# KRLabsOrg/verbatim-rag

Measured on AMD Instinct MI355X. Metric: query x chunk span-extractions/sec @512tok (ModernBERT-base extractor, chunks/s), higher is better.
Workload: dtype bf16

## Files before the change

### verbatim-rag_amd/csrc/qkv_attn.hip

```cpp
#include "qkv_attn.h"

#include <cstdlib>
#include <type_traits>

#ifdef VRAG_DEBUG_API
#define VRAG_DBG(bit) ((p.debug_flags & (bit)) != 0)
#else
#define VRAG_DBG(bit) false
#endif

namespace vrag {

constexpr int QA_WB = 192 * 128;
constexpr int QA_XOFF = 2 * QA_WB;
constexpr int QA_TAB = 131072;
constexpr int QA_MU = QA_TAB, QA_RS = QA_TAB + 2048, QA_LS = QA_TAB + 4096;
constexpr int QA_CA = QA_TAB + 5120, QA_SA = QA_CA + 4096, QA_CB = QA_SA + 4096, QA_SB = QA_CB + 2048;
constexpr int QA_SMEM = QA_SB + 2048;
constexpr int QA_V_OFF = 65536;

constexpr float QA_LAZY = 8.0f;
__device__ __forceinline__ float max3f(float a, float b, float c) { return __builtin_fmaxf(__builtin_fmaxf(a, b), c); }

template <int N>
__device__ __forceinline__ void wait_vm() {
  asm volatile("s_waitcnt vmcnt(%0)" ::"n"(N) : "memory");
}

template <bool LOCAL, bool FOLD, typename T>
__global__ __launch_bounds__(512, 2) void qkv_attn_kernel(const QkvAttnParams p) {
  typedef typename Op<T>::v4 V4;
  typedef typename Op<T>::v8 V8;
  extern __shared__ __attribute__((aligned(16))) char smem[];
  const int tid = threadIdx.x;
  const int lane = tid & 63;
  const int wave = uniform(tid >> 6);
  const int g = lane >> 4, l15 = lane & 15;
  const int H = p.H, Tp = p.Tp, nh = p.nh;
  const int xcd = blockIdx.x & 7, slot = blockIdx.x >> 3;
  const int grp = (slot / nh) * 8 + xcd, head = slot % nh;
  if (grp >= p.n_groups) return;
  const int4 wd = p.groups[grp * 8 + wave];
  const int wrow0 = uniform(wd.x), S = uniform(wd.y), kbase = uniform(wd.z);
  const int srow0 = wave * 64;
  const int qrow0 = (wave - kbase) * 64;
  const bool active = qrow0 < S;
  const T* X = reinterpret_cast<const T*>(p.x);
  const T* Wh = reinterpret_cast<const T*>(p.w) + (size_t)head * 192 * H;

  unsigned voffX[2], voffW[3];
#pragma unroll
  for (int par = 0; par < 2; ++par) {
    const int r = par * 8 + (lane >> 3);
    voffX[par] = (unsigned)(r * H + (((lane & 7) ^ ((r >> 1) & 7)) << 3)) * 2u;
  }
#pragma unroll
  for (int i = 0; i < 3; ++i) {
    const int row = wave * 24 + i * 8 + (lane >> 3);
    voffW[i] = (unsigned)(row * H + (((lane & 7) ^ ((row >> 1) & 7)) << 3)) * 2u;
  }
  const char* const Xw = reinterpret_cast<const char*>(X + (size_t)wrow0 * H);
  const char* const Wb = reinterpret_cast<const char*>(Wh);
  char* const xbuf = smem + QA_XOFF + wave * 8192;
  auto dma_w = [&](int kt, int buf, int i) {
    if (VRAG_DBG(4)) return;
    unsigned vo = voffW[i];
    asm volatile("" : "+v"(vo));
    glds16(Wb + kt * 128 + vo, smem + buf * QA_WB + (wave * 24 + i * 8) * 128);
  };
  auto dma_x = [&](int kt, int i) {
    if (!active || VRAG_DBG(4)) return;
    unsigned vo = voffX[i & 1];
    asm volatile("" : "+v"(vo));
    glds16(Xw + ((size_t)(i >> 1) * 16 * H + kt * 64) * 2 + vo, xbuf + i * 1024);
  };

  if (!VRAG_DBG(4)) {
    if (FOLD && lane < 16) {
      glds16(p.ln_mu + min(wrow0 + lane * 4, Tp - 4), smem + QA_MU + srow0 * 4);
      glds16(p.ln_rstd + min(wrow0 + lane * 4, Tp - 4), smem + QA_RS + srow0 * 4);
    }
    if (FOLD && wave == 2) glds16(p.ln_s + head * 192 + lane * 4, smem + QA_LS);
    if (wave == 2 || wave == 3) {
      const float* tab = wave == 2 ? p.rope_cos : p.rope_sin;
#pragma unroll
      for (int i = 0; i < 2; ++i) {
        const int r = i * 8 + (lane >> 3);
        glds16(tab + min(r, p.rope_rows - 1) * 32 + (((lane & 7) ^ ((r >> 1) & 7)) << 2), smem + (wave == 2 ? QA_CB : QA_SB) + i * 1024);
      }
    }
    if (wave == 4 || wave == 5) {
      const float* tab = wave == 4 ? p.rope_cos : p.rope_sin;
#pragma unroll
      for (int i = 0; i < 4; ++i)
        glds16(tab + (size_t)min(16 * (i * 8 + (lane >> 3)), p.rope_rows - 1) * 32 + (lane & 7) * 4, smem + (wave == 4 ? QA_CA : QA_SA) + i * 1024);
    }
  }

  f32x4 acc[12][4];
#pragma unroll
  for (int a = 0; a < 12; ++a)
#pragma unroll
    for (int c = 0; c < 4; ++c) acc[a][c] = f32x4{0.f, 0.f, 0.f, 0.f};

  const int KT = H >> 6;
  int fo[2];
#pragma unroll
  for (int s2 = 0; s2 < 2; ++s2) fo[s2] = l15 * 128 + ((((4 * s2 + g) ^ ((l15 >> 1) & 7))) << 4);
#ifdef VRAG_DEBUG_API
  const int probe = p.debug_flags;
#else
  int probe = 0;
  asm volatile("" : "+s"(probe));
#endif
  const bool mm = active && !(probe & 2);
#pragma unroll
  for (int i = 0; i < 3; ++i) dma_w(0, 0, i);
#pragma unroll
  for (int i = 0; i < 8; ++i) dma_x(0, i);
  for (int kt = 0; kt < KT; ++kt) {
    wait_vm<0>();
    __builtin_amdgcn_s_barrier();
    asm volatile("" ::: "memory");
    const char* sW = smem + (kt & 1) * QA_WB;
    const bool more = kt + 1 < KT;
    V8 xf[2][4], wa;
    if (mm) {
#pragma unroll
      for (int s2 = 0; s2 < 2; ++s2)
#pragma unroll
        for (int rt = 0; rt < 4; ++rt) xf[s2][rt] = *reinterpret_cast<const V8*>(xbuf + rt * 16 * 128 + fo[s2]);
      wa = *reinterpret_cast<const V8*>(sW + fo[0]);
    }
    asm volatile("s_waitcnt lgkmcnt(0)" ::: "memory");
    __builtin_amdgcn_sched_barrier(0);
    if (mm) {
#pragma unroll
      for (int it = 0; it < 24; ++it) {
        const int s2 = it / 12, nj = it % 12;
        V8 na = wa;
        if (it < 23) na = *reinterpret_cast<const V8*>(sW + ((it + 1) % 12) * 16 * 128 + fo[(it + 1) / 12]);
        __builtin_amdgcn_sched_barrier(0);
#pragma unroll
        for (int rt = 0; rt < 4; ++rt) {
          if (nj < 8) acc[nj][rt] = Op<T>::mfma16(wa, xf[s2][rt], acc[nj][rt]);
          else acc[nj][rt] = Op<T>::mfma16(xf[s2][rt], wa, acc[nj][rt]);
        }
        __builtin_amdgcn_sched_barrier(0);
        if (more && it < 11) {
          if (it < 3) dma_w(kt + 1, (kt + 1) & 1, it);
          else dma_x(kt + 1, it - 3);
        }
        __builtin_amdgcn_sched_barrier(0);
        wa = na;
      }
    } else if (more) {
#pragma unroll
      for (int i = 0; i < 3; ++i) dma_w(kt + 1, (kt + 1) & 1, i);
#pragma unroll
      for (int i = 0; i < 8; ++i) dma_x(kt + 1, i);
    }
  }
  __syncthreads();
  if (VRAG_DBG(16)) return;

  const float* l_mu = reinterpret_cast<const float*>(smem + QA_MU) + srow0;
  const float* l_rs = reinterpret_cast<const float*>(smem + QA_RS) + srow0;
  const float* l_ls = reinterpret_cast<const float*>(smem + QA_LS);
#pragma unroll
  for (int db = 0; db < 4; ++db) {
    const int d = db * 16 + l15;
    const float lsv = FOLD ? l_ls[128 + d] : 0.f;
#pragma unroll
    for (int tp = 0; tp < 2; ++tp) {
      V8 vv;
#pragma unroll
      for (int a = 0; a < 2; ++a) {
        const int rt = 2 * tp + a;
        f32x4 m4 = {0.f, 0.f, 0.f, 0.f}, r4 = {1.f, 1.f, 1.f, 1.f};
        if constexpr (FOLD) {
          m4 = *reinterpret_cast<const f32x4*>(l_mu + rt * 16 + 4 * g);
          r4 = *reinterpret_cast<const f32x4*>(l_rs + rt * 16 + 4 * g);
        }
#pragma unroll
        for (int h = 0; h < 2; ++h) {
          const int r0 = 2 * h;
          const f32x2 v = pk_fma(f32x2{-m4[r0], -m4[r0 + 1]}, splat2(lsv), f32x2{acc[8 + db][rt][r0], acc[8 + db][rt][r0 + 1]}) * f32x2{r4[r0], r4[r0 + 1]};
#pragma unroll
          for (int e = 0; e < 2; ++e)
            vv[a * 4 + r0 + e] = qrow0 + rt * 16 + 4 * g + r0 + e < S ? Op<T>::to(v[e]) : (T)0.f;
        }
      }
      const int c = wave * 8 + tp * 4 + g;
      *reinterpret_cast<V8*>(smem + QA_V_OFF + d * 1024 + ((c ^ l15) << 4)) = vv;
    }
  }
  auto rope_rows = [&](int a0, int rt, int ls_off, float scale, V8 (&out)[2]) {
    const bool live = qrow0 + rt * 16 + l15 < S;
    const float mu = FOLD ? l_mu[rt * 16 + l15] : 0.f, rs = FOLD ? l_rs[rt * 16 + l15] : 1.f;
#pragma unroll
    for (int np = 0; np < 2; ++np) {
      const int dd = np * 16 + 4 * g;
      const f32x4 ca = *reinterpret_cast<const f32x4*>(smem + QA_CA + (((qrow0 >> 4) + rt) * 32 + dd) * 4);
      const f32x4 sa = *reinterpret_cast<const f32x4*>(smem + QA_SA + (((qrow0 >> 4) + rt) * 32 + dd) * 4);
      const int bsw = l15 * 128 + ((((dd >> 2) ^ ((l15 >> 1) & 7))) << 4);
      const f32x4 cb = *reinterpret_cast<const f32x4*>(smem + QA_CB + bsw);
      const f32x4 sb = *reinterpret_cast<const f32x4*>(smem + QA_SB + bsw);
      f32x4 l1 = {0.f, 0.f, 0.f, 0.f}, l2 = {0.f, 0.f, 0.f, 0.f};
      if constexpr (FOLD) {
        l1 = *reinterpret_cast<const f32x4*>(l_ls + ls_off + dd);
        l2 = *reinterpret_cast<const f32x4*>(l_ls + ls_off + 32 + dd);
      }
#pragma unroll
      for (int h = 0; h < 2; ++h) {
        const int j0 = 2 * h;
        f32x2 x1 = {acc[a0 + np][rt][j0], acc[a0 + np][rt][j0 + 1]}, x2 = {acc[a0 + 2 + np][rt][j0], acc[a0 + 2 + np][rt][j0 + 1]};
        if constexpr (FOLD) {
          x1 = pk_fma(splat2(-mu), f32x2{l1[j0], l1[j0 + 1]}, x1) * rs;
          x2 = pk_fma(splat2(-mu), f32x2{l2[j0], l2[j0 + 1]}, x2) * rs;
        }
        const f32x2 ca2 = {ca[j0], ca[j0 + 1]}, sa2 = {sa[j0], sa[j0 + 1]}, cb2 = {cb[j0], cb[j0 + 1]}, sb2 = {sb[j0], sb[j0 + 1]};
        const f32x2 c = pk_fma(-sa2, sb2, ca2 * cb2), sn = pk_fma(ca2, sb2, sa2 * cb2);
        const f32x2 o1 = pk_fma(-x2, sn, x1 * c) * scale, o2 = pk_fma(x1, sn, x2 * c) * scale;
#pragma unroll
        for (int e = 0; e < 2; ++e) {
          if constexpr (!std::is_same<T, bf16_t>::value) {
            out[0][np * 4 + j0 + e] = live ? Op<T>::to(o1[e]) : (T)0.f;
            out[1][np * 4 + j0 + e] = live ? Op<T>::to(o2[e]) : (T)0.f;
          } else {
            out[0][np * 4 + j0 + e] = Op<T>::to(o1[e]);
            out[1][np * 4 + j0 + e] = Op<T>::to(o2[e]);
          }
        }
      }
    }
  };
#pragma unroll
  for (int rt = 0; rt < 4; ++rt) {
    V8 kf[2];
    rope_rows(4, rt, 64, 1.0f, kf);
    const int row = srow0 + rt * 16 + l15;
#pragma unroll
    for (int s = 0; s < 2; ++s) *reinterpret_cast<V8*>(smem + row * 128 + (((4 * s + g) ^ ((row >> 1) & 7)) << 4)) = kf[s];
  }
  V8 qf[4][2];
#pragma unroll
  for (int rt = 0; rt < 4; ++rt) rope_rows(0, rt, 0, p.q_scale, qf[rt]);
  __syncthreads();

  f32x4 ot[4][4];
  f32x4 lo[4];
#pragma unroll
  for (int c = 0; c < 4; ++c) {
    lo[c] = f32x4{0.f, 0.f, 0.f, 0.f};
#pragma unroll
    for (int dt = 0; dt < 4; ++dt) ot[c][dt] = f32x4{0.f, 0.f, 0.f, 0.f};
  }
  float m_run[4] = {0.f, 0.f, 0.f, 0.f};
  bool seen[4] = {false, false, false, false};
  V8 ones;
#pragma unroll
  for (int j = 0; j < 8; ++j) ones[j] = (T)1.0f;
  const int W = p.window;
  int kt_lo = 0, kt_hi = (S - 1) >> 6;
  if constexpr (LOCAL) {
    kt_lo = max(0, qrow0 - W) >> 6;
    kt_hi = min(S - 1, qrow0 + 63 + W) >> 6;
  }
  const int ksw = (l15 >> 1) & 7;
  if (active && !VRAG_DBG(1)) {
    for (int kt = kt_lo; kt <= kt_hi; ++kt) {
      bool cut[2][2];
#pragma unroll
      for (int u = 0; u < 2; ++u) {
        const int q_lo = qrow0 + 32 * u;
#pragma unroll
        for (int t2 = 0; t2 < 2; ++t2) {
          const int kh = kt * 64 + t2 * 32;
          bool outside = kh >= S || q_lo >= S;
          cut[u][t2] = kh + 31 >= S;
          if constexpr (LOCAL) {
            outside = outside || (kh + 31 < q_lo - W) || (kh > q_lo + 31 + W);
            cut[u][t2] = cut[u][t2] || (kh < q_lo + 31 - W) || (kh + 31 > q_lo + W);
          }
          cut[u][t2] = cut[u][t2] || outside;
        }
      }
      V8 pf[4][2];
      {
        f32x4 st[4][4];
#pragma unroll
        for (int c = 0; c < 4; ++c) {
          const float seed = -m_run[c];
#pragma unroll
          for (int kb = 0; kb < 4; ++kb) st[c][kb] = f32x4{seed, seed, seed, seed};
        }
#pragma unroll
        for (int kb = 0; kb < 4; ++kb) {
          const char* krow = smem + ((kbase + kt) * 64 + kb * 16 + l15) * 128;
          const V8 k0 = *reinterpret_cast<const V8*>(krow + ((g ^ ksw) << 4));
          const V8 k1 = *reinterpret_cast<const V8*>(krow + (((4 + g) ^ ksw) << 4));
#pragma unroll
          for (int c = 0; c < 4; ++c) {
            st[c][kb] = Op<T>::mfma16(k0, qf[c][0], st[c][kb]);
            st[c][kb] = Op<T>::mfma16(k1, qf[c][1], st[c][kb]);
          }
        }
        float mx[4];
#pragma unroll
        for (int c = 0; c < 4; ++c) {
          const int u = c >> 1;
          mx[c] = -INFINITY;
#pragma unroll
          for (int t2 = 0; t2 < 2; ++t2) {
            if (cut[u][t2]) {
              const int qi = qrow0 + 16 * c + l15;
              int lo_k = 0, hi_k = S - 1;
              if constexpr (LOCAL) {
                lo_k = max(0, qi - W);
                hi_k = min(S - 1, qi + W);
              }
              const unsigned span = hi_k >= lo_k ? (unsigned)(hi_k - lo_k) : 0u;
              int d0 = hi_k >= lo_k ? kt * 64 + t2 * 32 + 4 * g - lo_k : -100000;
              asm volatile("" : "+v"(d0));
#pragma unroll
              for (int h2 = 0; h2 < 2; ++h2)
#pragma unroll
                for (int r = 0; r < 4; ++r) {
                  const bool ok = (unsigned)(d0 + 16 * h2 + r) <= span;
                  st[c][2 * t2 + h2][r] = ok ? st[c][2 * t2 + h2][r] : -INFINITY;
                }
            }
            const f32x4& a = st[c][2 * t2];
            const f32x4& b2 = st[c][2 * t2 + 1];
            mx[c] = max3f(mx[c], max3f(a[0], a[1], a[2]), max3f(a[3], b2[0], b2[1]));
            mx[c] = max3f(mx[c], b2[2], b2[3]);
          }
        }
        bool move = false;
#pragma unroll
        for (int c = 0; c < 4; ++c) move = move || mx[c] > QA_LAZY || (!seen[c] && mx[c] > -INFINITY);
        if (__any(move)) {
#pragma unroll
          for (int c = 0; c < 4; ++c) {
            float m_all = fmaxf(mx[c], __shfl_xor(mx[c], 16, 64));
            m_all = fmaxf(m_all, __shfl_xor(m_all, 32, 64));
            const bool has = m_all > -INFINITY;
            const float delta = seen[c] ? fmaxf(m_all, 0.f) : (has ? m_all : 0.f);
            const float alpha = seen[c] ? __builtin_amdgcn_exp2f(-delta) : 1.0f;
            seen[c] = seen[c] || has;
            m_run[c] += delta;
#pragma unroll
            for (int kb = 0; kb < 4; ++kb)
#pragma unroll
              for (int r = 0; r < 4; ++r) st[c][kb][r] -= delta;
#pragma unroll
            for (int dt = 0; dt < 4; ++dt)
#pragma unroll
              for (int r = 0; r < 4; ++r) ot[c][dt][r] *= alpha;
#pragma unroll
            for (int r = 0; r < 4; ++r) lo[c][r] *= alpha;
          }
        }
#pragma unroll
        for (int c = 0; c < 4; ++c)
#pragma unroll
          for (int t2 = 0; t2 < 2; ++t2)
#pragma unroll
            for (int j = 0; j < 8; ++j) pf[c][t2][j] = (T)__builtin_amdgcn_exp2f(st[c][2 * t2 + (j >> 2)][j & 3]);
      }
#pragma unroll
      for (int t2 = 0; t2 < 2; ++t2) {
#pragma unroll
        for (int c = 0; c < 4; ++c) lo[c] = Op<T>::mfma16(ones, pf[c][t2], lo[c]);
#pragma unroll
        for (int dt = 0; dt < 4; ++dt) {
          const V8 vf = *reinterpret_cast<const V8*>(smem + QA_V_OFF + (dt * 16 + l15) * 1024 + ((((kbase + kt) * 8 + t2 * 4 + g) ^ l15) << 4));
#pragma unroll
          for (int c = 0; c < 4; ++c) ot[c][dt] = Op<T>::mfma16(vf, pf[c][t2], ot[c][dt]);
        }
      }
    }
  }
  __syncthreads();

  if (active) {
    char* stg = smem + wave * 8192;
#pragma unroll
    for (int rt = 0; rt < 4; ++rt) {
      const int row = rt * 16 + l15;
      const bool live = qrow0 + row < S;
      const float inv = live ? 1.0f / lo[rt][0] : 0.f;
#pragma unroll
      for (int db = 0; db < 4; ++db) {
        V4 o;
#pragma unroll
        for (int j = 0; j < 4; ++j) o[j] = live ? Op<T>::to(ot[rt][db][j] * inv) : (T)0.f;
        const int c16 = db * 2 + (g >> 1);
        *reinterpret_cast<V4*>(stg + row * 128 + ((c16 ^ (row & 7)) << 4) + ((g & 1) << 3)) = o;
      }
    }
#pragma unroll
    for (int it = 0; it < 8; ++it) {
      const int row = it * 8 + (lane >> 3), c16 = lane & 7;
      const f32x4 v = *reinterpret_cast<const f32x4*>(stg + row * 128 + ((c16 ^ (row & 7)) << 4));
      if (qrow0 + row < S && !VRAG_DBG(8)) store16_nt(reinterpret_cast<T*>(p.o) + (size_t)(wrow0 + row) * H + head * 64 + c16 * 8, v);
    }
  }
}

template <bool LOCAL, bool FOLD, typename T>
static hipError_t launch_t(const QkvAttnParams& p, hipStream_t stream) {
  static bool attr = false;
  if (!attr) {
    hipError_t e = hipFuncSetAttribute(reinterpret_cast<const void*>(&qkv_attn_kernel<LOCAL, FOLD, T>),
                                       hipFuncAttributeMaxDynamicSharedMemorySize, QA_SMEM);
    if (e != hipSuccess) return e;
    attr = true;
  }
  const int grid = ((p.n_groups + 7) / 8) * 8 * p.nh;
  hipLaunchKernelGGL((qkv_attn_kernel<LOCAL, FOLD, T>), dim3(grid), dim3(512), QA_SMEM, stream, p);
  return hipGetLastError();
}

hipError_t launch_qkv_attention(const QkvAttnParams& p, bool local, hipStream_t stream) {
  if (p.n_groups <= 0) return hipSuccess;
  if (p.H % 64 != 0 || p.H != p.nh * 64 || (size_t)p.Tp * p.H >= (size_t)1 << 31) return hipErrorInvalidValue;
  const bool fold = p.ln_mu != nullptr;
  if (p.op_dtype == kOpF16) {
    if (fold) return local ? launch_t<true, true, f16_t>(p, stream) : launch_t<false, true, f16_t>(p, stream);
    return local ? launch_t<true, false, f16_t>(p, stream) : launch_t<false, false, f16_t>(p, stream);
  }
  if (fold) return local ? launch_t<true, true, bf16_t>(p, stream) : launch_t<false, true, bf16_t>(p, stream);
  return local ? launch_t<true, false, bf16_t>(p, stream) : launch_t<false, false, bf16_t>(p, stream);
}

__global__ void permute_qkv_heads_kernel(const bf16_t* __restrict__ w, const float* __restrict__ s, int H, int nh,
                                         bf16_t* __restrict__ w_out, float* __restrict__ s_out) {
  const int orow = blockIdx.x;
  const int head = orow / 192, part = (orow % 192) / 64, d = orow % 64;
  const int src = part * H + head * 64 + d;
  for (int i = threadIdx.x; i < H; i += blockDim.x) w_out[(size_t)orow * H + i] = w[(size_t)src * H + i];
  if (threadIdx.x == 0 && s && s_out) s_out[orow] = s[src];
}

hipError_t permute_qkv_heads(const bf16_t* w, const float* s, int H, int nh, bf16_t* w_out, float* s_out, hipStream_t stream) {
  hipLaunchKernelGGL(permute_qkv_heads_kernel, dim3(3 * H), dim3(256), 0, stream, w, s, H, nh, w_out, s_out);
  return hipGetLastError();
}

int fused_pack_groups(const int* seq_row, const int* seq_len, int seq0, int seq1, int4* out) {
  int n = 0, used = 8;
  for (int s = seq0; s < seq1; ++s) {
    const int need = (seq_len[s] + 63) / 64;
    if (used + need > 8) {
      for (int w = 0; w < 8; ++w) out[n * 8 + w] = int4{0, 0, 0, 0};
      ++n;
      used = 0;
    }
    for (int j = 0; j < need; ++j) out[(n - 1) * 8 + used + j] = int4{seq_row[s] + 64 * j, seq_len[s], used, 0};
    used += need;
  }
  return n;
}

unsigned qkv_attn_f16_saturated(bool reset) { return f16_sat_take(reset); }
unsigned* qkv_attn_f16_flag_address() { return f16_sat_flag_address(); }

}
```

Baseline: 7860.

## Skip dead 32x32 sub-tiles at local-window edges and merge Q/K RoPE passes

The key-tile loop becomes a templated tile lambda that takes a compile-time live mask. For local attention, the first and last key tiles are peeled off and run with masks that drop MFMA, softmax and PV work for 32x32 quadrants wholly outside the window. Separately, RoPE for K and Q now runs in one pass per row tile, sharing the cos/sin table loads. Risks include more code size and register pressure from the extra instantiations, and the asm barrier on qf may change scheduling.

```diff
diff --git a/verbatim-rag_amd/csrc/qkv_attn.hip b/verbatim-rag_amd/csrc/qkv_attn.hip
--- a/verbatim-rag_amd/csrc/qkv_attn.hip
+++ b/verbatim-rag_amd/csrc/qkv_attn.hip
@@ -195,7 +195,7 @@
       *reinterpret_cast<V8*>(smem + QA_V_OFF + d * 1024 + ((c ^ l15) << 4)) = vv;
     }
   }
-  auto rope_rows = [&](int a0, int rt, int ls_off, float scale, V8 (&out)[2]) {
+  auto rope_rows = [&](int rt, V8 (&kout)[2], V8 (&qout)[2]) {
     const bool live = qrow0 + rt * 16 + l15 < S;
     const float mu = FOLD ? l_mu[rt * 16 + l15] : 0.f, rs = FOLD ? l_rs[rt * 16 + l15] : 1.f;
 #pragma unroll
@@ -206,46 +206,49 @@
       const int bsw = l15 * 128 + ((((dd >> 2) ^ ((l15 >> 1) & 7))) << 4);
       const f32x4 cb = *reinterpret_cast<const f32x4*>(smem + QA_CB + bsw);
       const f32x4 sb = *reinterpret_cast<const f32x4*>(smem + QA_SB + bsw);
-      f32x4 l1 = {0.f, 0.f, 0.f, 0.f}, l2 = {0.f, 0.f, 0.f, 0.f};
-      if constexpr (FOLD) {
-        l1 = *reinterpret_cast<const f32x4*>(l_ls + ls_off + dd);
-        l2 = *reinterpret_cast<const f32x4*>(l_ls + ls_off + 32 + dd);
-      }
 #pragma unroll
       for (int h = 0; h < 2; ++h) {
         const int j0 = 2 * h;
-        f32x2 x1 = {acc[a0 + np][rt][j0], acc[a0 + np][rt][j0 + 1]}, x2 = {acc[a0 + 2 + np][rt][j0], acc[a0 + 2 + np][rt][j0 + 1]};
-        if constexpr (FOLD) {
-          x1 = pk_fma(splat2(-mu), f32x2{l1[j0], l1[j0 + 1]}, x1) * rs;
-          x2 = pk_fma(splat2(-mu), f32x2{l2[j0], l2[j0 + 1]}, x2) * rs;
-        }
         const f32x2 ca2 = {ca[j0], ca[j0 + 1]}, sa2 = {sa[j0], sa[j0 + 1]}, cb2 = {cb[j0], cb[j0 + 1]}, sb2 = {sb[j0], sb[j0 + 1]};
         const f32x2 c = pk_fma(-sa2, sb2, ca2 * cb2), sn = pk_fma(ca2, sb2, sa2 * cb2);
-        const f32x2 o1 = pk_fma(-x2, sn, x1 * c) * scale, o2 = pk_fma(x1, sn, x2 * c) * scale;
-#pragma unroll
-        for (int e = 0; e < 2; ++e) {
-          if constexpr (!std::is_same<T, bf16_t>::value) {
-            out[0][np * 4 + j0 + e] = live ? Op<T>::to(o1[e]) : (T)0.f;
-            out[1][np * 4 + j0 + e] = live ? Op<T>::to(o2[e]) : (T)0.f;
-          } else {
-            out[0][np * 4 + j0 + e] = Op<T>::to(o1[e]);
-            out[1][np * 4 + j0 + e] = Op<T>::to(o2[e]);
+#pragma unroll
+        for (int part = 0; part < 2; ++part) {
+          const int a0 = part ? 0 : 4, ls_off = part ? 0 : 64;
+          const float scale = part ? p.q_scale : 1.0f;
+          V8(&out)[2] = part ? qout : kout;
+          f32x2 x1 = {acc[a0 + np][rt][j0], acc[a0 + np][rt][j0 + 1]}, x2 = {acc[a0 + 2 + np][rt][j0], acc[a0 + 2 + np][rt][j0 + 1]};
+          if constexpr (FOLD) {
+            const f32x2 l1 = *reinterpret_cast<const f32x2*>(l_ls + ls_off + dd + j0);
+            const f32x2 l2 = *reinterpret_cast<const f32x2*>(l_ls + ls_off + 32 + dd + j0);
+            x1 = pk_fma(splat2(-mu), l1, x1) * rs;
+            x2 = pk_fma(splat2(-mu), l2, x2) * rs;
           }
+          const f32x2 o1 = pk_fma(-x2, sn, x1 * c) * scale, o2 = pk_fma(x1, sn, x2 * c) * scale;
+#pragma unroll
+          for (int e = 0; e < 2; ++e) {
+            if constexpr (!std::is_same<T, bf16_t>::value) {
+              out[0][np * 4 + j0 + e] = live ? Op<T>::to(o1[e]) : (T)0.f;
+              out[1][np * 4 + j0 + e] = live ? Op<T>::to(o2[e]) : (T)0.f;
+            } else {
+              out[0][np * 4 + j0 + e] = Op<T>::to(o1[e]);
+              out[1][np * 4 + j0 + e] = Op<T>::to(o2[e]);
+            }
+          }
         }
       }
     }
   };
+  V8 qf[4][2];
 #pragma unroll
   for (int rt = 0; rt < 4; ++rt) {
     V8 kf[2];
-    rope_rows(4, rt, 64, 1.0f, kf);
+    rope_rows(rt, kf, qf[rt]);
     const int row = srow0 + rt * 16 + l15;
 #pragma unroll
     for (int s = 0; s < 2; ++s) *reinterpret_cast<V8*>(smem + row * 128 + (((4 * s + g) ^ ((row >> 1) & 7)) << 4)) = kf[s];
-  }
-  V8 qf[4][2];
-#pragma unroll
-  for (int rt = 0; rt < 4; ++rt) rope_rows(0, rt, 0, p.q_scale, qf[rt]);
+#pragma unroll
+    for (int s = 0; s < 2; ++s) asm volatile("" : "+v"(qf[rt][s]));
+  }
   __syncthreads();
 
   f32x4 ot[4][4];
@@ -268,119 +271,149 @@
     kt_hi = min(S - 1, qrow0 + 63 + W) >> 6;
   }
   const int ksw = (l15 >> 1) & 7;
+  auto tile = [&](int kt, auto live_c) __attribute__((always_inline)) {
+    constexpr int LIVE = decltype(live_c)::value;
+    constexpr auto on = [](int u, int t2) { return ((LIVE >> (2 * u + t2)) & 1) != 0; };
+    bool cut[2][2];
+#pragma unroll
+    for (int u = 0; u < 2; ++u) {
+      const int q_lo = qrow0 + 32 * u;
+#pragma unroll
+      for (int t2 = 0; t2 < 2; ++t2) {
+        const int kh = kt * 64 + t2 * 32;
+        cut[u][t2] = kh + 31 >= S || q_lo >= S;
+        if constexpr (LOCAL) cut[u][t2] = cut[u][t2] || (kh < q_lo + 31 - W) || (kh + 31 > q_lo + W);
+      }
+    }
+    V8 pf[4][2];
+    {
+      f32x4 st[4][4];
+#pragma unroll
+      for (int c = 0; c < 4; ++c) {
+        const float seed = -m_run[c];
+#pragma unroll
+        for (int kb = 0; kb < 4; ++kb) st[c][kb] = f32x4{seed, seed, seed, seed};
+      }
+#pragma unroll
+      for (int kb = 0; kb < 4; ++kb) {
+        if (!on(0, kb >> 1) && !on(1, kb >> 1)) continue;
+        const char* krow = smem + ((kbase + kt) * 64 + kb * 16 + l15) * 128;
+        const V8 k0 = *reinterpret_cast<const V8*>(krow + ((g ^ ksw) << 4));
+        const V8 k1 = *reinterpret_cast<const V8*>(krow + (((4 + g) ^ ksw) << 4));
+#pragma unroll
+        for (int c = 0; c < 4; ++c) {
+          if (!on(c >> 1, kb >> 1)) continue;
+          st[c][kb] = Op<T>::mfma16(k0, qf[c][0], st[c][kb]);
+          st[c][kb] = Op<T>::mfma16(k1, qf[c][1], st[c][kb]);
+        }
+      }
+      float mx[4];
+#pragma unroll
+      for (int c = 0; c < 4; ++c) {
+        const int u = c >> 1;
+        mx[c] = -INFINITY;
+#pragma unroll
+        for (int t2 = 0; t2 < 2; ++t2) {
+          if (!on(u, t2)) continue;
+          if (cut[u][t2]) {
+            const int qi = qrow0 + 16 * c + l15;
+            int lo_k = 0, hi_k = S - 1;
+            if constexpr (LOCAL) {
+              lo_k = max(0, qi - W);
+              hi_k = min(S - 1, qi + W);
+            }
+            const unsigned span = hi_k >= lo_k ? (unsigned)(hi_k - lo_k) : 0u;
+            int d0 = hi_k >= lo_k ? kt * 64 + t2 * 32 + 4 * g - lo_k : -100000;
+            asm volatile("" : "+v"(d0));
+#pragma unroll
+            for (int h2 = 0; h2 < 2; ++h2)
+#pragma unroll
+              for (int r = 0; r < 4; ++r) {
+                const bool ok = (unsigned)(d0 + 16 * h2 + r) <= span;
+                st[c][2 * t2 + h2][r] = ok ? st[c][2 * t2 + h2][r] : -INFINITY;
+              }
+          }
+          const f32x4& a = st[c][2 * t2];
+          const f32x4& b2 = st[c][2 * t2 + 1];
+          mx[c] = max3f(mx[c], max3f(a[0], a[1], a[2]), max3f(a[3], b2[0], b2[1]));
+          mx[c] = max3f(mx[c], b2[2], b2[3]);
+        }
+      }
+      bool move = false;
+#pragma unroll
+      for (int c = 0; c < 4; ++c) move = move || mx[c] > QA_LAZY || (!seen[c] && mx[c] > -INFINITY);
+      if (__any(move)) {
+#pragma unroll
+        for (int c = 0; c < 4; ++c) {
+          float m_all = fmaxf(mx[c], __shfl_xor(mx[c], 16, 64));
+          m_all = fmaxf(m_all, __shfl_xor(m_all, 32, 64));
+          const bool has = m_all > -INFINITY;
+          const float delta = seen[c] ? fmaxf(m_all, 0.f) : (has ? m_all : 0.f);
+          const float alpha = seen[c] ? __builtin_amdgcn_exp2f(-delta) : 1.0f;
+          seen[c] = seen[c] || has;
+          m_run[c] += delta;
+#pragma unroll
+          for (int kb = 0; kb < 4; ++kb)
+#pragma unroll
+            for (int r = 0; r < 4; ++r) st[c][kb][r] -= delta;
+#pragma unroll
+          for (int dt = 0; dt < 4; ++dt)
+#pragma unroll
+            for (int r = 0; r < 4; ++r) ot[c][dt][r] *= alpha;
+#pragma unroll
+          for (int r = 0; r < 4; ++r) lo[c][r] *= alpha;
+        }
+      }
+#pragma unroll
+      for (int c = 0; c < 4; ++c)
+#pragma unroll
+        for (int t2 = 0; t2 < 2; ++t2) {
+          if (!on(c >> 1, t2)) continue;
+#pragma unroll
+          for (int j = 0; j < 8; ++j) pf[c][t2][j] = (T)__builtin_amdgcn_exp2f(st[c][2 * t2 + (j >> 2)][j & 3]);
+        }
+    }
+#pragma unroll
+    for (int t2 = 0; t2 < 2; ++t2) {
+      if (!on(0, t2) && !on(1, t2)) continue;
+#pragma unroll
+      for (int c = 0; c < 4; ++c)
+        if (on(c >> 1, t2)) lo[c] = Op<T>::mfma16(ones, pf[c][t2], lo[c]);
+#pragma unroll
+      for (int dt = 0; dt < 4; ++dt) {
+        const V8 vf = *reinterpret_cast<const V8*>(smem + QA_V_OFF + (dt * 16 + l15) * 1024 + ((((kbase + kt) * 8 + t2 * 4 + g) ^ l15) << 4));
+#pragma unroll
+        for (int c = 0; c < 4; ++c)
+          if (on(c >> 1, t2)) ot[c][dt] = Op<T>::mfma16(vf, pf[c][t2], ot[c][dt]);
+      }
+    }
+  };
+  auto live_mask = [&](int kt) {
+    int live = 0;
+#pragma unroll
+    for (int u = 0; u < 2; ++u)
+#pragma unroll
+      for (int t2 = 0; t2 < 2; ++t2) {
+        const int q_lo = qrow0 + 32 * u, kh = kt * 64 + t2 * 32;
+        bool outside = kh >= S || q_lo >= S;
+        if constexpr (LOCAL) outside = outside || (kh + 31 < q_lo - W) || (kh > q_lo + 31 + W);
+        live |= outside ? 0 : 1 << (2 * u + t2);
+      }
+    return live;
+  };
   if (active && !VRAG_DBG(1)) {
-    for (int kt = kt_lo; kt <= kt_hi; ++kt) {
-      bool cut[2][2];
-#pragma unroll
-      for (int u = 0; u < 2; ++u) {
-        const int q_lo = qrow0 + 32 * u;
-#pragma unroll
-        for (int t2 = 0; t2 < 2; ++t2) {
-          const int kh = kt * 64 + t2 * 32;
-          bool outside = kh >= S || q_lo >= S;
-          cut[u][t2] = kh + 31 >= S;
-          if constexpr (LOCAL) {
-            outside = outside || (kh + 31 < q_lo - W) || (kh > q_lo + 31 + W);
-            cut[u][t2] = cut[u][t2] || (kh < q_lo + 31 - W) || (kh + 31 > q_lo + W);
-          }
-          cut[u][t2] = cut[u][t2] || outside;
-        }
-      }
-      V8 pf[4][2];
-      {
-        f32x4 st[4][4];
-#pragma unroll
-        for (int c = 0; c < 4; ++c) {
-          const float seed = -m_run[c];
-#pragma unroll
-          for (int kb = 0; kb < 4; ++kb) st[c][kb] = f32x4{seed, seed, seed, seed};
-        }
-#pragma unroll
-        for (int kb = 0; kb < 4; ++kb) {
-          const char* krow = smem + ((kbase + kt) * 64 + kb * 16 + l15) * 128;
-          const V8 k0 = *reinterpret_cast<const V8*>(krow + ((g ^ ksw) << 4));
-          const V8 k1 = *reinterpret_cast<const V8*>(krow + (((4 + g) ^ ksw) << 4));
-#pragma unroll
-          for (int c = 0; c < 4; ++c) {
-            st[c][kb] = Op<T>::mfma16(k0, qf[c][0], st[c][kb]);
-            st[c][kb] = Op<T>::mfma16(k1, qf[c][1], st[c][kb]);
-          }
-        }
-        float mx[4];
-#pragma unroll
-        for (int c = 0; c < 4; ++c) {
-          const int u = c >> 1;
-          mx[c] = -INFINITY;
-#pragma unroll
-          for (int t2 = 0; t2 < 2; ++t2) {
-            if (cut[u][t2]) {
-              const int qi = qrow0 + 16 * c + l15;
-              int lo_k = 0, hi_k = S - 1;
-              if constexpr (LOCAL) {
-                lo_k = max(0, qi - W);
-                hi_k = min(S - 1, qi + W);
-              }
-              const unsigned span = hi_k >= lo_k ? (unsigned)(hi_k - lo_k) : 0u;
-              int d0 = hi_k >= lo_k ? kt * 64 + t2 * 32 + 4 * g - lo_k : -100000;
-              asm volatile("" : "+v"(d0));
-#pragma unroll
-              for (int h2 = 0; h2 < 2; ++h2)
-#pragma unroll
-                for (int r = 0; r < 4; ++r) {
-                  const bool ok = (unsigned)(d0 + 16 * h2 + r) <= span;
-                  st[c][2 * t2 + h2][r] = ok ? st[c][2 * t2 + h2][r] : -INFINITY;
-                }
-            }
-            const f32x4& a = st[c][2 * t2];
-            const f32x4& b2 = st[c][2 * t2 + 1];
-            mx[c] = max3f(mx[c], max3f(a[0], a[1], a[2]), max3f(a[3], b2[0], b2[1]));
-            mx[c] = max3f(mx[c], b2[2], b2[3]);
-          }
-        }
-        bool move = false;
-#pragma unroll
-        for (int c = 0; c < 4; ++c) move = move || mx[c] > QA_LAZY || (!seen[c] && mx[c] > -INFINITY);
-        if (__any(move)) {
-#pragma unroll
-          for (int c = 0; c < 4; ++c) {
-            float m_all = fmaxf(mx[c], __shfl_xor(mx[c], 16, 64));
-            m_all = fmaxf(m_all, __shfl_xor(m_all, 32, 64));
-            const bool has = m_all > -INFINITY;
-            const float delta = seen[c] ? fmaxf(m_all, 0.f) : (has ? m_all : 0.f);
-            const float alpha = seen[c] ? __builtin_amdgcn_exp2f(-delta) : 1.0f;
-            seen[c] = seen[c] || has;
-            m_run[c] += delta;
-#pragma unroll
-            for (int kb = 0; kb < 4; ++kb)
-#pragma unroll
-              for (int r = 0; r < 4; ++r) st[c][kb][r] -= delta;
-#pragma unroll
-            for (int dt = 0; dt < 4; ++dt)
-#pragma unroll
-              for (int r = 0; r < 4; ++r) ot[c][dt][r] *= alpha;
-#pragma unroll
-            for (int r = 0; r < 4; ++r) lo[c][r] *= alpha;
-          }
-        }
-#pragma unroll
-        for (int c = 0; c < 4; ++c)
-#pragma unroll
-          for (int t2 = 0; t2 < 2; ++t2)
-#pragma unroll
-            for (int j = 0; j < 8; ++j) pf[c][t2][j] = (T)__builtin_amdgcn_exp2f(st[c][2 * t2 + (j >> 2)][j & 3]);
-      }
-#pragma unroll
-      for (int t2 = 0; t2 < 2; ++t2) {
-#pragma unroll
-        for (int c = 0; c < 4; ++c) lo[c] = Op<T>::mfma16(ones, pf[c][t2], lo[c]);
-#pragma unroll
-        for (int dt = 0; dt < 4; ++dt) {
-          const V8 vf = *reinterpret_cast<const V8*>(smem + QA_V_OFF + (dt * 16 + l15) * 1024 + ((((kbase + kt) * 8 + t2 * 4 + g) ^ l15) << 4));
-#pragma unroll
-          for (int c = 0; c < 4; ++c) ot[c][dt] = Op<T>::mfma16(vf, pf[c][t2], ot[c][dt]);
-        }
-      }
-    }
+    int kt0 = kt_lo, kt1 = kt_hi;
+    bool left = false, right = false;
+    if constexpr (LOCAL) {
+      left = kt0 < kt1 && (live_mask(kt0) & ~0xB) == 0;
+      right = kt0 < kt1 && (live_mask(kt1) & ~0xD) == 0;
+      kt0 += left;
+      kt1 -= right;
+      if (left) tile(kt_lo, std::integral_constant<int, 0xB>{});
+    }
+    for (int kt = kt0; kt <= kt1; ++kt) tile(kt, std::integral_constant<int, 0xF>{});
+    if constexpr (LOCAL)
+      if (right) tile(kt_hi, std::integral_constant<int, 0xD>{});
   }
   __syncthreads();
 
```

Result: no change. 7933, median of 6 (+0.9%).
